# HamidGadirov/OpticalFlowSciVis

Measured on AMD Instinct MI355X. Metric: volume-pairs/sec, Flow-3D unsupervised train step (fwd+loss+bwd+AdamW), higher is better.
Workload: dtype f32

## Files before the change

### opticalflowscivis_amd/csrc/convtr.hip

```cpp
#include <cstdint>
#include <cstdlib>

#include "common.hpp"

namespace {

typedef float f32x16 __attribute__((ext_vector_type(16)));

struct TP {
  int B, Cin, Cout;
  int CoutT;
  int Di, Hi, Wi;
  int Dout, Hout, Wout;
  int Dq, Hq, Wq;
  int tz, ty, tx;
  long long tiles;
  const float* slope;
  float* Z;
  int nslope;
  const float* addend;
  const float* Ybase;
  long long wslice;
#ifdef FS_ABLATION
  int ab = 0;
// ... 568 lines not shown
#pragma unroll
    for (int cls = 0; cls < 8; ++cls) {
      const int pz = cls >> 2, py = (cls >> 1) & 1, px = cls & 1;
#pragma unroll
      for (int tp = 0; tp < 8; ++tp) {
        const int a = tp >> 2, bb = (tp >> 1) & 1, c = tp & 1;
        const int kidx = (tap_k(pz, a) * 4 + tap_k(py, bb)) * 4 + tap_k(px, c);
        const int didx = ((tap_d(pz, a) + 1) * 3 + (tap_d(py, bb) + 1)) * 3 + (tap_d(px, c) + 1);
        const float av = aB[kidx * 16];
#pragma unroll
        for (int n = 0; n < 2; ++n)
          acc[n][cls] = __builtin_amdgcn_mfma_f32_16x16x4f32(av, xn[n][didx], acc[n][cls], 0, 0, 0);
      }
    }
    __builtin_amdgcn_s_barrier();
    buf ^= 1;
  }

#ifdef FS_ABLATION
  if (p.ab & 4) return;
#endif
  const int qz = qz0 + wz, qy = qy0 + wy;
  if (qz < p.Dq && qy < p.Hq) {
    const size_t yvol = (size_t)p.Dout * p.Hout * p.Wout;
#pragma unroll
    for (int n = 0; n < 2; ++n) {
      const int qx = qx0 + 16 * n + col;
#pragma unroll
      for (int r = 0; r < 4; ++r) {
        const int co = 4 * kq + r;
        const bool ok = co < p.Cout;
        const int cc = ok ? co : 0;
        const float bv = (bias && ok) ? bias[cc] : 0.f;
        float v[8];
#pragma unroll
        for (int c = 0; c < 8; ++c) v[c] = acc[n][c][r] + bv;
        store8_quad(Y + ((size_t)b * p.Cout + cc) * yvol, v, qz, qy, qx, ok, p,
                    p.Z ? p.Z + ((size_t)b * p.Cout + cc) * yvol : nullptr, p.Z ? p.slope[p.nslope == 1 ? 0 : cc] : 0.f);
      }
    }
  }
}

constexpr int p8_ws_ci(int rt) { return 128 * rt + 16; }
__host__ __device__ constexpr int p8_k(int par, int d) { return par == 0 ? (d == 0 ? 1 : 3) : (d == 0 ? 0 : 2); }

#ifdef FS_TR_STAMPS
__device__ unsigned long long fs_tr_dbg[4 * 8];
#define TSTAMP(i) do { const unsigned long long now_ = __builtin_amdgcn_s_memtime(); dt[i] += now_ - tprev; tprev = now_; } while (0)
#else
#define TSTAMP(i) do { } while (0)
#endif

template <int RT, int NT, int CINP>
__global__ __launch_bounds__(512, 2) void convtr_p8_kernel(const float* __restrict__ X, const float* __restrict__ Wt,
                                                        const float* __restrict__ bias, float* __restrict__ Y,
                                                        TP p, int per) {
  constexpr int CI = 4, XB = 16 * (NT - 1);
  constexpr int ZT = 3, YT = 3, XP = XB + 16;
  constexpr int PS = YT * XP;
  constexpr int CHS = ZT * PS + ((ZT * PS) % 32 == 16 ? 0 : 16);
  constexpr int NX = CI * CHS;
  constexpr int NXL = (NX + 255) / 256 * 256;
  constexpr int WSCI = p8_ws_ci(RT);
  constexpr int NW = CINP * WSCI;
  constexpr int NWL = (NW + 255) / 256 * 256;
  static_assert((NWL + 2 * NXL) * 4 <= 160 * 1024, "weights + two input buffers fit the CU's LDS");
  static_assert(NT % 2 == 1, "tiles are processed in pairs + one");
  __shared__ __attribute__((aligned(16))) float lds[NWL + 2 * NXL];

  const int t = threadIdx.x, lane = t & 63;
  const int wave = __builtin_amdgcn_readfirstlane(t >> 6);
  const int wv = wave & 3;
  const long long t0 = (long long)blockIdx.x * per, t1 = min(t0 + per, p.tiles);
  const size_t xvol = (size_t)p.Di * p.Hi * p.Wi;
  auto decode = [&](long long tile, int& b, int& qz0, int& qy0, int& q0) {
    const int txi = (int)(tile % p.tx); tile /= p.tx;
    const int tyi = (int)(tile % p.ty); tile /= p.ty;
    const int tzi = (int)(tile % p.tz);
    b = (int)(tile / p.tz);
    qz0 = tzi * 2; qy0 = tyi * 2; q0 = txi * XB;
  };

  if (wave >= 4) {
#if defined(__HIP_DEVICE_COMPILE__)
    __builtin_amdgcn_s_setprio(3);
    constexpr int NXW = (NXL / 256 + 3) / 4, NWW = (NWL / 256 + 3) / 4;
    {
      __amdgpu_buffer_rsrc_t rw = __builtin_amdgcn_make_buffer_rsrc((void*)Wt, (short)0, (p.Cin + 3) / 4 * 4 * WSCI * 4,
                                                                     0x00020000);
#pragma unroll
      for (int k = 0; k < NWW; ++k)
        if (256 * (wv + 4 * k) < NWL)
          __builtin_amdgcn_raw_ptr_buffer_load_lds(rw, (lds_ptr_t)(lds + 256 * (wv + 4 * k)), 16,
                                                   (unsigned)(256 * (wv + 4 * k) + 4 * lane) * 4u, 0, 0, 0);
    }
    unsigned xoff[NXW];
    int b = 0;
    auto offsets = [&](long long tile) {
      int qz0, qy0, q0;
      decode(tile, b, qz0, qy0, q0);
#pragma unroll
      for (int k = 0; k < NXW; ++k) {
        const int i = 256 * (wv + 4 * k) + 4 * lane;
        const int c = i / CHS, r1 = i - c * CHS;
        const int z = r1 / PS, r2 = r1 - z * PS;
        const int y = r2 / XP, x = r2 - y * XP;
        const int gz = qz0 - 1 + z, gy = qy0 - 1 + y, gx = q0 - 4 + x;
        const bool ok = i < NX && z < ZT && gz >= 0 && gz < p.Di && gy >= 0 && gy < p.Hi && gx >= 0 && gx < p.Wi;
        xoff[k] = ok ? ((unsigned)c * (unsigned)xvol + ((unsigned)gz * p.Hi + gy) * p.Wi + gx) * 4u : DMA_OOB;
// ... 47 lines not shown
  for (long long tile = t0; tile < t1; ++tile) {
    int b, qz0, qy0, q0;
    decode(tile, b, qz0, qy0, q0);
    const int qend = (q0 + XB >= p.Wi) ? p.Wi + 1 : q0 + XB;
    f32x4 acc[RT][NT];
#pragma unroll
    for (int rt = 0; rt < RT; ++rt)
#pragma unroll
      for (int n = 0; n < NT; ++n)
#pragma unroll
        for (int r = 0; r < 4; ++r) acc[rt][n][r] = 0.f;

    for (int c0 = 0; c0 < p.Cin; c0 += CI) {
      const float* aB = lds + (size_t)(c0 + kq) * WSCI + col;
      float av[8][RT];
#pragma unroll
      for (int d = 0; d < 8; ++d)
#pragma unroll
        for (int rt = 0; rt < RT; ++rt) av[d][rt] = aB[(d * RT + rt) * 16];
      const float* bB = lds + bBo + buf * NXL;
      float xa[2][8], xb[2][8];
      auto load_x = [&](int n, float (&xn)[8]) {
#pragma unroll
        for (int d = 0; d < 8; ++d) xn[d] = bB[16 * n - ((d >> 2) & 1) * PS - ((d >> 1) & 1) * XP - (d & 1)];
      };
      auto mma_pair = [&](int n, const float (&x0)[8], const float (&x1)[8], bool two) {
#pragma unroll
        for (int d = 0; d < 8; ++d)
#pragma unroll
          for (int rt = 0; rt < RT; ++rt) {
            acc[rt][n] = __builtin_amdgcn_mfma_f32_16x16x4f32(av[d][rt], x0[d], acc[rt][n], 0, 0, 0);
            if (two) acc[rt][n + 1] = __builtin_amdgcn_mfma_f32_16x16x4f32(av[d][rt], x1[d], acc[rt][n + 1], 0, 0, 0);
          }
      };
      load_x(0, xa[0]);
      if (NT > 1) load_x(1, xa[1]);
#pragma unroll
      for (int n = 0; n < NT; n += 4) {
        if (n + 2 < NT) { load_x(n + 2, xb[0]); if (n + 3 < NT) load_x(n + 3, xb[1]); }
        __builtin_amdgcn_sched_barrier(0);
        mma_pair(n, xa[0], xa[1], n + 1 < NT);
        if (n + 2 < NT) {
          if (n + 4 < NT) { load_x(n + 4, xa[0]); if (n + 5 < NT) load_x(n + 5, xa[1]); }
          __builtin_amdgcn_sched_barrier(0);
          mma_pair(n + 2, xb[0], xb[1], n + 3 < NT);
        }
      }
      TSTAMP(0);
      __builtin_amdgcn_s_barrier();
      TSTAMP(1);
      buf ^= 1;
    }

    const int qz = qz0 + wz, qy = qy0 + wy;
    if (qz <= p.Di && qy <= p.Hi) {
      const size_t yvol = (size_t)p.Dout * p.Hout * p.Wout;
      const bool evn = (col & 1) == 0;
      const int slot = 4 * (kq & 1) + (evn ? 0 : 1) + 2 * (lane >> 5);
#pragma unroll
      for (int rt = 0; rt < RT; ++rt) {
        const int item = 8 * rt + slot;
        const int pzy = item / p.Cout, co = item - pzy * p.Cout;
        const int zo = 2 * qz - (pzy >> 1), yo = 2 * qy - (pzy & 1);
        const bool iok = item < 4 * p.Cout && zo >= 0 && zo < p.Dout && yo >= 0 && yo < p.Hout;
        const float bv = (bias && iok) ? bias[co] : 0.f;
        float* __restrict__ row = Y + (((size_t)b * p.Cout + (iok ? co : 0)) * p.Dout + (iok ? zo : 0)) * ((size_t)p.Hout * p.Wout) +
                                  (size_t)(iok ? yo : 0) * p.Wout;
        const float* __restrict__ arow = p.addend ? p.addend + (row - Y) : nullptr;
        (void)yvol;
        float4 apre[NT];
        if (arow != nullptr) {
#pragma unroll
          for (int n = 0; n < NT; ++n) {
            const int qa = evn ? q0 + 16 * n + col : q0 + 16 * n + col - 1;
            const int x0 = 2 * qa - 1;
            const bool full = iok && qa >= 1 && qa + 1 < qend && x0 + 3 < p.Wout;
            apre[n] = full ? *reinterpret_cast<const float4*>(arow + x0) : make_float4(0.f, 0.f, 0.f, 0.f);
          }
        }
#pragma unroll
        for (int n = 0; n < NT; ++n) {
          const int q = q0 + 16 * n + col;
          const auto s0 = __builtin_amdgcn_permlane32_swap(__float_as_uint(acc[rt][n][0]), __float_as_uint(acc[rt][n][2]),
                                                           false, false);
          const auto s1 = __builtin_amdgcn_permlane32_swap(__float_as_uint(acc[rt][n][1]), __float_as_uint(acc[rt][n][3]),
                                                           false, false);
          const unsigned keep_e = evn ? s0[0] : s1[0], keep_o = evn ? s0[1] : s1[1];
          const unsigned send_e = evn ? s1[0] : s0[0], send_o = evn ? s1[1] : s0[1];
          const float re = __uint_as_float(__builtin_amdgcn_update_dpp(0u, send_e, 0xB1, 0xF, 0xF, false)) + bv;
          const float ro = __uint_as_float(__builtin_amdgcn_update_dpp(0u, send_o, 0xB1, 0xF, 0xF, false)) + bv;
          const float ke = __uint_as_float(keep_e) + bv, ko = __uint_as_float(keep_o) + bv;
          const int qa = evn ? q : q - 1;
          float4 v = evn ? make_float4(ko, ke, ro, re) : make_float4(ro, re, ko, ke);
          if (iok) {
            const int x0 = 2 * qa - 1;
            const bool full = qa >= 1 && qa + 1 < qend && x0 + 3 < p.Wout;
            if (full) {
              if (arow) { v.x += apre[n].x; v.y += apre[n].y; v.z += apre[n].z; v.w += apre[n].w; }
              *reinterpret_cast<float4*>(row + x0) = v;
            } else {
              const float vv[4] = {v.x, v.y, v.z, v.w};
#pragma unroll
              for (int e = 0; e < 4; ++e) {
                const int x = x0 + e, pos = qa + (e >> 1);
                if (pos >= 0 && pos < qend && x >= 0 && x < p.Wout) row[x] = vv[e] + (arow ? arow[x] : 0.f);
              }
            }
          }
        }
      }
    }
    TSTAMP(2);
  }
#ifdef FS_TR_STAMPS
  if (blockIdx.x == 3 && lane == 0) {
    for (int i = 0; i < 8; ++i) fs_tr_dbg[wv * 8 + i] = dt[i];
    fs_tr_dbg[wv * 8 + 7] = (unsigned long long)(t1 - t0);
  }
#endif
}

static int tr_ncu() {
  static int ncu_of[64] = {};
  int dev = 0;
  if (hipGetDevice(&dev) != hipSuccess || dev < 0 || dev >= 64) dev = 0;
  int ncu = ncu_of[dev];
  if (ncu == 0) {
    int n = 0;
    if (hipDeviceGetAttribute(&n, hipDeviceAttributeMultiprocessorCount, dev) != hipSuccess || n < 1) n = 256;
    ncu_of[dev] = ncu = n;
  }
  return ncu;
}

template <int RT, int NT, int CINP = 32>
void launch_p8(const float* x, const float* ws, const float* bias, float* y, const TP& p, hipStream_t st) {
  const int ncu = tr_ncu();
  const long long nwg = p.tiles < ncu ? p.tiles : ncu;
  const int per = (int)((p.tiles + nwg - 1) / nwg);
  const unsigned grid = (unsigned)((p.tiles + per - 1) / per);
  hipLaunchKernelGGL((convtr_p8_kernel<RT, NT, CINP>), dim3(grid), dim3(512), 0, st, x, ws, bias, y, p, per);
}

template <int CO, int NP>
__global__ __launch_bounds__(256) void convtr_valu_kernel(const float* __restrict__ X, const float* __restrict__ W,
                                                          const float* __restrict__ bias, float* __restrict__ Y,
                                                          TP p) {
  const int Hq2 = (p.Hq + NP - 1) / NP;
  const long long nq = (long long)p.B * p.Dq * Hq2 * p.Wq;
  const long long e = (long long)blockIdx.x * 256 + threadIdx.x;
  if (e >= nq) return;
  const int qx = (int)(e % p.Wq);
  long long r = e / p.Wq;
  const int qy = (int)(r % Hq2) * NP; r /= Hq2;
  const int qz = (int)(r % p.Dq);
  const int b = (int)(r / p.Dq);

  constexpr int NY = NP + 2;
  int off[3 * NY * 3];
#pragma unroll
  for (int dz = 0; dz < 3; ++dz)
#pragma unroll
    for (int dy = 0; dy < NY; ++dy)
#pragma unroll
      for (int dx = 0; dx < 3; ++dx) {
        const int z = qz + dz - 1, y = qy + dy - 1, x = qx + dx - 1;
        const bool ok = z >= 0 && z < p.Di && y >= 0 && y < p.Hi && x >= 0 && x < p.Wi;
        off[(dz * NY + dy) * 3 + dx] = ok ? (z * p.Hi + y) * p.Wi + x : -1;
      }

  float acc[NP][CO][8];
#pragma unroll
// ... 13 lines not shown
    const float* wc = W + (size_t)ci * p.Cout * 64;
#pragma unroll
    for (int co = 0; co < CO; ++co) {
      if (co < p.Cout) {
#pragma unroll
        for (int cls = 0; cls < 8; ++cls) {
          const int pz = cls >> 2, py = (cls >> 1) & 1, px = cls & 1;
#pragma unroll
          for (int tp = 0; tp < 8; ++tp) {
            const int a = tp >> 2, bb = (tp >> 1) & 1, c = tp & 1;
            const int kidx = (tap_k(pz, a) * 4 + tap_k(py, bb)) * 4 + tap_k(px, c);
            const float wv = wc[co * 64 + kidx];
#pragma unroll
            for (int q = 0; q < NP; ++q) {
              const int didx = ((tap_d(pz, a) + 1) * NY + (tap_d(py, bb) + 1 + q)) * 3 + (tap_d(px, c) + 1);
              acc[q][co][cls] = fmaf(xn[didx], wv, acc[q][co][cls]);
            }
          }
        }
      }
    }
  }
  const size_t yvol = (size_t)p.Dout * p.Hout * p.Wout;
#pragma unroll
  for (int q = 0; q < NP; ++q)
#pragma unroll
    for (int co = 0; co < CO; ++co)
      if (co < p.Cout && qy + q < p.Hq)
        store8(Y + ((size_t)b * p.Cout + co) * yvol, acc[q][co], qz, qy + q, qx, p,
               p.Z ? p.Z + ((size_t)b * p.Cout + co) * yvol : nullptr, p.Z ? p.slope[p.nslope == 1 ? 0 : co] : 0.f);
}

template <int CO>
void launch_valu(const float* x, const float* w, const float* bias, float* y, const TP& p, hipStream_t st) {
  constexpr int NP = 2;
  const long long nq = (long long)p.B * p.Dq * ((p.Hq + NP - 1) / NP) * p.Wq;
  hipLaunchKernelGGL((convtr_valu_kernel<CO, NP>), dim3((unsigned)((nq + 255) / 256)), dim3(256), 0, st, x, w, bias,
                     y, p);
}

}

#ifdef FS_TR_STAMPS
extern "C" int fs_debug_tr_stamps(unsigned long long* out) {
  return hipMemcpyFromSymbol(out, HIP_SYMBOL(fs_tr_dbg), sizeof(unsigned long long) * 32) == hipSuccess ? 0 : 1;
}
#endif

extern "C" long long fs_conv3d_tr_ws_floats(int Cin, int Cout) {
  if (Cin < 1 || Cout < 1 || (Cout > 32 && (Cout % 32 != 0 || Cout > 128))) return -1;
  const int slices = Cout > 32 ? Cout / 32 : 1;
  if (Cout > 32) Cout = 32;
  const long long cinp = (Cin + 3) / 4 * 4;
  const long long p8 = Cout <= 12 ? cinp * p8_ws_ci(Cout <= 2 ? 1 : (Cout <= 6 ? 3 : 6)) : 0;
  long long cls = Cout <= 6 ? 0 : cinp * 64 * (Cout <= 16 ? 16 : 32);
  if (Cout > 16 && t3_slab_words(Cin) > cls) cls = t3_slab_words(Cin);
  if (Cout <= 16 && t3_slab_words16(Cin) > cls) cls = t3_slab_words16(Cin);
  return (p8 > cls ? p8 : cls) * slices;
}

static int conv3d_tr_slice(const float* x, const float* w, const float* bias, const float* slope, int nslope,
                          const float* addend, float* y, float* z, float* ws, int B, int Cin, int Cout, int Di,
                          int Hi, int Wi, int Dout, int Hout, int Wout, fs_stream_t stream, int CoutT = 0, int slices = 1,
                          WprepPlan* plan = nullptr) {
  FS_REQUIRE_PTR(x);
  if (plan == nullptr) FS_REQUIRE_PTR(y);
  if (z != nullptr && (slope == nullptr || (nslope != 1 && nslope != Cout))) return FS_ERR_ARG;
  if (B < 1 || Cin < 1 || Cout < 1 || Di < 1 || Hi < 1 || Wi < 1) return FS_ERR_SHAPE;
  if (Cout > 32) return FS_ERR_ARG;
  if (CoutT == 0) CoutT = Cout;
  if ((Dout != 2 * Di && Dout != 2 * Di + 1) || (Hout != 2 * Hi && Hout != 2 * Hi + 1) ||
      (Wout != 2 * Wi && Wout != 2 * Wi + 1))
    return FS_ERR_SHAPE;
  if ((long long)Di * Hi * Wi >= (1ll << 31) || (long long)Dout * Hout * Wout >= (1ll << 31))
    return FS_ERR_SHAPE;
  if ((long long)4 * Di * Hi * Wi * 4 >= (1ll << 32)) return FS_ERR_SHAPE;
  TP p;
  p.B = B; p.Cin = Cin; p.Cout = Cout; p.CoutT = CoutT; p.Di = Di; p.Hi = Hi; p.Wi = Wi;
  p.Dout = Dout; p.Hout = Hout; p.Wout = Wout;
  p.Dq = (Dout + 1) / 2; p.Hq = (Hout + 1) / 2; p.Wq = (Wout + 1) / 2;
  p.slope = slope; p.Z = z; p.nslope = nslope;
  p.addend = addend; p.Ybase = y;
  p.wslice = 0;
  hipStream_t st = (hipStream_t)stream;
  if ((long long)B * p.Dq * p.Hq * p.Wq >= (1ll << 31) * 256) return FS_ERR_SHAPE;
  static const bool reg_only = FS_AB_ENV("FLOWSCI_TR_REG");
  static const bool p8_all = FS_AB_ENV("FLOWSCI_TR_P8_ALL");
  static const bool s3_small = FS_AB_ENV("FLOWSCI_TR_S3_SMALL");
  if (!s3_small && Cout <= (p8_all ? 12 : 6) && !reg_only && z == nullptr && ws != nullptr && Cin <= (Cout <= 6 ? 64 : 32) && Dout == 2 * Di && Hout == 2 * Hi &&
      Wout == 2 * Wi && Wi % 4 == 0 && (((uintptr_t)x | (uintptr_t)ws) & 15) == 0 &&
      (long long)4 * Di * Hi * Wi * 4 < (1ll << 31)) {
    const int rt = Cout <= 2 ? 1 : (Cout <= 6 ? 3 : 6);
    const bool wide = Wi > 64 && rt < 6;
    p.tz = fs::cdiv(Di + 1, 2); p.ty = fs::cdiv(Hi + 1, 2); p.tx = fs::cdiv(Wi, wide ? 128 : 64);
    p.tiles = (long long)B * p.tz * p.ty * p.tx;
    if (p.tiles >= 16 && p.tiles < (1ll << 31)) {
      const int cinp = (Cin + 3) / 4 * 4;
      wprep_do(wprep_job(FS_WPREP_P8, w, ws, (long long)cinp * p8_ws_ci(rt), Cin, Cout, cinp, rt), plan, st);
      if (plan != nullptr) return FS_OK;
      if (Cin > 32) {
        if (rt == 1) { if (wide) launch_p8<1, 9, 64>(x, ws, bias, y, p, st); else launch_p8<1, 5, 64>(x, ws, bias, y, p, st); }
        else { if (wide) launch_p8<3, 9, 64>(x, ws, bias, y, p, st); else launch_p8<3, 5, 64>(x, ws, bias, y, p, st); }
      } else if (rt == 1) { if (wide) launch_p8<1, 9>(x, ws, bias, y, p, st); else launch_p8<1, 5>(x, ws, bias, y, p, st); }
      else if (rt == 3) { if (wide) launch_p8<3, 9>(x, ws, bias, y, p, st); else launch_p8<3, 5>(x, ws, bias, y, p, st); }
      else launch_p8<6, 5>(x, ws, bias, y, p, st);
      FS_LAUNCH_CHECK();
      return FS_OK;
    }
  }
  if (Cout <= 6 && !s3_small) {
    if (plan != nullptr) return FS_OK;
    if (w == nullptr) return FS_ERR_NULLPTR;
    if (Cout == 1) launch_valu<1>(x, w, bias, y, p, st);
    else if (Cout <= 2) launch_valu<2>(x, w, bias, y, p, st);
    else if (Cout <= 4) launch_valu<4>(x, w, bias, y, p, st);
    else launch_valu<6>(x, w, bias, y, p, st);
    FS_LAUNCH_CHECK();
    return FS_OK;
  }
  FS_REQUIRE_PTR(ws);
  const int cinp = (Cin + 3) / 4 * 4;
  p.tz = fs::cdiv(p.Dq, 2); p.ty = fs::cdiv(p.Hq, 2); p.tx = fs::cdiv(p.Wq, 32);
  p.tiles = (long long)B * p.tz * p.ty * p.tx;
  if (p.tiles >= (1ll << 31)) return FS_ERR_SHAPE;
#ifdef FS_ABLATION
  static const int tr_ab = (int)FS_AB_ENV_LL("FLOWSCI_TR_AB", 0);
  p.ab = tr_ab;
#endif
  const bool ws_ok = !reg_only && Wi % 4 == 0 && (((uintptr_t)x | (uintptr_t)ws) & 15) == 0 && p.tiles * slices >= 128 &&
                     (long long)4 * Di * Hi * Wi * 4 < (1ll << 31);
  static const bool no_s3 = FS_AB_ENV("FLOWSCI_TR_NO_S3");
  const long long t3 = (long long)B * fs::cdiv(Di, T3_TZ) * fs::cdiv(Hi, T3_TY) * fs::cdiv(Wi, T3_TW);
  const bool t3_ok = !no_s3 && !reg_only && Dout == 2 * Di && Hout == 2 * Hi && Wout == 2 * Wi && Wi % 4 == 0 &&
                     (((uintptr_t)x | (uintptr_t)ws) & 15) == 0 && (long long)Di * Hi * Wi * 4 < (1ll << 31) &&
                     t3 * slices >= 256 && t3 < (1ll << 31) && (long long)32 * Dout * Hout * Wout * 4 < (1ll << 32);
  if (Cout <= 16) {
    if (t3_ok && slices == 1) {
      wprep_do(wprep_job(FS_WPREP_TRS3_16, w, ws, t3_slab_words16(Cin), Cin, Cout, (Cin + 3) / 4, p.CoutT), plan, st);
      if (plan != nullptr) return FS_OK;
      p.tz = fs::cdiv(Di, T3_TZ); p.ty = fs::cdiv(Hi, T3_TY); p.tx = fs::cdiv(Wi, T3_TW);
      p.tiles = t3;
      const int ncu = tr_ncu();
      const long long gx = ncu < p.tiles ? ncu : p.tiles;
      hipLaunchKernelGGL(convtr_s3_kernel<true>, dim3((unsigned)gx, 1), dim3(64 * (T3_NMW + T3_NLW)), 0, st, x,
                         reinterpret_cast<const unsigned*>(ws), bias, y, p);
      FS_LAUNCH_CHECK();
      return FS_OK;
    }
    wprep_do(wprep_job(FS_WPREP_TR16, w, ws, (long long)cinp * 64 * 16, Cin, Cout, cinp), plan, st);
    if (plan != nullptr) return FS_OK;
    if (ws_ok)
// ... 85 lines not shown
```

### opticalflowscivis_amd/csrc/wprep.hpp

```cpp
#pragma once

enum { FS_WPREP_FWD = 0, FS_WPREP_TR32 = 1, FS_WPREP_TR16 = 2, FS_WPREP_P8 = 3, FS_WPREP_WINO = 4, FS_WPREP_WINO4 = 5,
       FS_WPREP_WINO2D = 6, FS_WPREP_S3K4 = 7, FS_WPREP_TRS3 = 8, FS_WPREP_TRS3_16 = 9 };

__device__ __forceinline__ unsigned s3_pack(float a, float b) {
  typedef __bf16 bf16x2_t __attribute__((ext_vector_type(2)));
  const bf16x2_t h = {(__bf16)a, (__bf16)b};
  return __builtin_bit_cast(unsigned, h);
}

__device__ __forceinline__ unsigned wprep_s3_word(const FsWprepJob& j, int e) {
  const int Cout = j.p[0], Cin = j.p[1], CinP2 = j.p[2], CP = j.p[3];
  const float* __restrict__ w = j.w;
  const int kx = e & 3;
  int r = e >> 2;
  const int col = r % CP; r /= CP;
  const int kh = r & 1, kyp = (r >> 1) & 1; r >>= 2;
  const int piece = r % 3; r /= 3;
  const int kz = r & 3; r >>= 2;
  const int cp = r % CinP2, mg = r / CinP2;
  const int co = mg * CP + col, tap = (kz * 4 + 2 * kyp + kh) * 4 + kx;
  float v[2];
#pragma unroll
  for (int i = 0; i < 2; ++i) {
    const int ci = 2 * cp + i;
    float a = (co < Cout && ci < Cin) ? w[((size_t)co * Cin + ci) * 64 + tap] : 0.f;
    for (int q = 0; q < piece; ++q) a = a - (float)(__bf16)a;
    v[i] = a;
  }
  return s3_pack(v[0], v[1]);
}
__host__ __device__ constexpr int wprep_p8_k(int par, int d) { return par == 0 ? (d == 0 ? 1 : 3) : (d == 0 ? 0 : 2); }

__device__ __forceinline__ unsigned wprep_t3_word(const FsWprepJob& j, int e) {
  const int Cin = j.p[0], Cout = j.p[1], CoutT = j.p[3];
  const float* __restrict__ w = j.w;
  const int c2 = e & 1, dxa = (e >> 1) & 1, co = (e >> 2) & 31, kh = (e >> 7) & 1;
  int r = e >> 8;
  const int piece = r % 3; r /= 3;
  const int az = r & 1, cls = (r >> 1) & 7, st = r >> 4;
  const int pz = cls >> 2, py = (cls >> 1) & 1, px = cls & 1;
  const int tap = (wprep_p8_k(pz, az) * 4 + wprep_p8_k(py, kh)) * 4 + wprep_p8_k(px, 1 - dxa);
  float v[2];
#pragma unroll
  for (int i = 0; i < 2; ++i) {
    const int ci = 4 * st + 2 * c2 + i;
    float a = (co < Cout && ci < Cin) ? w[((size_t)ci * CoutT + co) * 64 + tap] : 0.f;
    for (int q = 0; q < piece; ++q) a = a - (float)(__bf16)a;
    v[i] = a;
  }
  return s3_pack(v[0], v[1]);
}
__device__ __forceinline__ unsigned wprep_t3_word16(const FsWprepJob& j, int e) {
  const int Cin = j.p[0], Cout = j.p[1], CoutT = j.p[3];
  const float* __restrict__ w = j.w;
  const int c2 = e & 1, az = (e >> 1) & 1, co = (e >> 2) & 15, kq = (e >> 6) & 3;
  int r = e >> 8;
  const int piece = r % 3; r /= 3;
  const int cls = r & 7, st = r >> 3;
  const int pz = cls >> 2, py = (cls >> 1) & 1, px = cls & 1;
  const int tap = (wprep_p8_k(pz, az) * 4 + wprep_p8_k(py, kq >> 1)) * 4 + wprep_p8_k(px, kq & 1);
  float v[2];
#pragma unroll
  for (int i = 0; i < 2; ++i) {
    const int ci = 4 * st + 2 * c2 + i;
    float a = (co < Cout && ci < Cin) ? w[((size_t)ci * CoutT + co) * 64 + tap] : 0.f;
    for (int q = 0; q < piece; ++q) a = a - (float)(__bf16)a;
    v[i] = a;
  }
  return s3_pack(v[0], v[1]);
}
constexpr int FS_WINO_UCH = 9 * 4 * 64 + 16;
constexpr int FS_WINO4_UCH = 9 * 6 * 64;
constexpr int FS_WINO2D_UCH = 3 * 24 * 64;

__device__ __forceinline__ float wprep_g43(const float (&g)[3], int tt) {
  switch (tt) {
    case 0: return 0.25f * g[0];
    case 1: return (-1.f / 6.f) * ((g[0] + g[2]) + g[1]);
    case 2: return (-1.f / 6.f) * ((g[0] + g[2]) - g[1]);
    case 3: return (1.f / 24.f) * g[0] + ((1.f / 12.f) * g[1] + (1.f / 6.f) * g[2]);
    case 4: return (1.f / 24.f) * g[0] + ((-1.f / 12.f) * g[1] + (1.f / 6.f) * g[2]);
    default: return g[2];
  }
}
// ... 16 lines not shown
    }
    case FS_WPREP_TR16: {
      const int Cin = j.p[0], Cout = j.p[1];
      const int co = e & 15, tap = (e >> 4) & 63, ci = e >> 10;
      return (co < Cout && ci < Cin) ? w[((size_t)ci * Cout + co) * 64 + tap] : 0.f;
    }
    case FS_WPREP_WINO: {
      const int Cout = j.p[0], Cin = j.p[1], mode = j.p[3];
      const int ci = e / FS_WINO_UCH, i = e - ci * FS_WINO_UCH;
      if (i >= 9 * 4 * 64 || ci >= Cin) return 0.f;
      const int kk = i >> 8, tt = (i >> 6) & 3, co = i & 63;
      if (co >= Cout) return 0.f;
      float g[3];
#pragma unroll
      for (int kx = 0; kx < 3; ++kx)
        g[kx] = mode ? w[((size_t)ci * Cout + co) * 27 + (26 - (kk * 3 + kx))] : w[((size_t)co * Cin + ci) * 27 + kk * 3 + kx];
      return tt == 0 ? g[0] : tt == 1 ? 0.5f * ((g[0] + g[1]) + g[2]) : tt == 2 ? 0.5f * ((g[0] - g[1]) + g[2]) : g[2];
    }
    case FS_WPREP_WINO4: {
      const int Cout = j.p[0], Cin = j.p[1], mode = j.p[3];
      const int ci = e / FS_WINO4_UCH, i = e - ci * FS_WINO4_UCH;
      if (ci >= Cin) return 0.f;
      const int kk = i / 384, r = i - kk * 384;
      const int tt = r >> 6, co = r & 63;
      if (co >= Cout) return 0.f;
      float g[3];
#pragma unroll
      for (int kx = 0; kx < 3; ++kx)
        g[kx] = mode ? w[((size_t)ci * Cout + co) * 27 + (26 - (kk * 3 + kx))] : w[((size_t)co * Cin + ci) * 27 + kk * 3 + kx];
      return wprep_g43(g, tt);
    }
    case FS_WPREP_WINO2D: {
      const int Cout = j.p[0], Cin = j.p[1], mode = j.p[3];
      const int ci = e / FS_WINO2D_UCH, i = e - ci * FS_WINO2D_UCH;
      if (ci >= Cin) return 0.f;
      const int kz = i / 1536, r = i - kz * 1536;
      const int ty = r / 384, r2 = r - ty * 384;
      const int tx = r2 >> 6, co = r2 & 63;
      if (co >= Cout) return 0.f;
      float u[3];
#pragma unroll
      for (int ky = 0; ky < 3; ++ky) {
        float g[3];
#pragma unroll
        for (int kx = 0; kx < 3; ++kx) {
          const int tap = (kz * 3 + ky) * 3 + kx;
          g[kx] = mode ? w[((size_t)ci * Cout + co) * 27 + (26 - tap)] : w[((size_t)co * Cin + ci) * 27 + tap];
        }
        u[ky] = wprep_g43(g, tx);
      }
      return ty == 0 ? u[0] : ty == 1 ? 0.5f * ((u[0] + u[1]) + u[2]) : ty == 2 ? 0.5f * ((u[0] - u[1]) + u[2]) : u[2];
    }
    default: {
      const int Cin = j.p[0], Cout = j.p[1], RT = j.p[3];
      const int wsci = 128 * RT + 16;
      const int ci = e / wsci, i = e - ci * wsci;
      if (i >= 128 * RT || ci >= Cin) return 0.f;
      const int d = i / (16 * RT), r2 = i - d * 16 * RT;
      const int rt = r2 >> 4, row = r2 & 15;
      const int px = row >> 3, item = 8 * rt + (row & 7);
      if (item >= 4 * Cout) return 0.f;
      const int pzy = item / Cout, co = item - pzy * Cout;
      const int kz = wprep_p8_k(pzy >> 1, (d >> 2) & 1), ky = wprep_p8_k(pzy & 1, (d >> 1) & 1), kx = wprep_p8_k(px, d & 1);
      return w[((size_t)ci * Cout + co) * 64 + (kz * 4 + ky) * 4 + kx];
    }
  }
}

__device__ __forceinline__ void wprep_wino2d_blocks(const FsWprepJob& j, int first, int stride) {
  __shared__ float g9[64 * 9 + 64];
  const int Cout = j.p[0], Cin = j.p[1], CinP = j.p[2], mode = j.p[3];
  const float* __restrict__ w = j.w;
  const int t = threadIdx.x;
  for (int blk = first; blk < CinP * 3; blk += stride) {
    const int ci = blk / 3, kz = blk - ci * 3;
    __syncthreads();
    for (int i = t; i < 64 * 9; i += 256) {
      const int co = i / 9, k9 = i - co * 9;
      const int tap = kz * 9 + k9;
      float v = 0.f;
      if (co < Cout && ci < Cin) v = mode ? w[((size_t)ci * Cout + co) * 27 + (26 - tap)] : w[((size_t)co * Cin + ci) * 27 + tap];
      g9[co * 10 + k9] = v;
    }
    __syncthreads();
    const int co = t & 63, q = t >> 6;
    float* __restrict__ dst = j.ws + (size_t)ci * FS_WINO2D_UCH + kz * 1536 + co;
#pragma unroll
    for (int k = 0; k < 6; ++k) {
      const int e = 6 * q + k, ty = e / 6, tx = e - ty * 6;
      float u[3];
#pragma unroll
      for (int ky = 0; ky < 3; ++ky) {
        const float g[3] = {g9[co * 10 + ky * 3], g9[co * 10 + ky * 3 + 1], g9[co * 10 + ky * 3 + 2]};
        u[ky] = wprep_g43(g, tx);
      }
      const float v = ty == 0 ? u[0] : ty == 1 ? 0.5f * ((u[0] + u[1]) + u[2]) : ty == 2 ? 0.5f * ((u[0] - u[1]) + u[2]) : u[2];
      dst[ty * 384 + tx * 64] = (co < Cout && ci < Cin) ? v : 0.f;
    }
  }
}

__global__ __launch_bounds__(256) void wprep_one_kernel(FsWprepJob j) {
  if (j.kind == FS_WPREP_WINO2D && j.total == j.p[2] * FS_WINO2D_UCH) {
    wprep_wino2d_blocks(j, blockIdx.x, gridDim.x);
    return;
  }
  if (j.kind == FS_WPREP_S3K4 || j.kind == FS_WPREP_TRS3 || j.kind == FS_WPREP_TRS3_16) {
    for (int e = blockIdx.x * 256 + threadIdx.x; e < j.total; e += gridDim.x * 256)
      reinterpret_cast<unsigned*>(j.ws)[e] = j.kind == FS_WPREP_S3K4 ? wprep_s3_word(j, e)
                                             : (j.kind == FS_WPREP_TRS3 ? wprep_t3_word(j, e) : wprep_t3_word16(j, e));
    return;
  }
  for (int e = blockIdx.x * 256 + threadIdx.x; e < j.total; e += gridDim.x * 256) j.ws[e] = wprep_elem(j, e);
}

__global__ __launch_bounds__(256) void wprep_batch_kernel(const FsWprepJob* __restrict__ jobs) {
  const FsWprepJob j = jobs[blockIdx.y];
  if (j.kind == FS_WPREP_WINO2D && j.total == j.p[2] * FS_WINO2D_UCH) {
    wprep_wino2d_blocks(j, blockIdx.x, gridDim.x);
    return;
  }
  if (j.kind == FS_WPREP_S3K4 || j.kind == FS_WPREP_TRS3 || j.kind == FS_WPREP_TRS3_16) {
    for (int e = blockIdx.x * 256 + threadIdx.x; e < j.total; e += gridDim.x * 256)
      reinterpret_cast<unsigned*>(j.ws)[e] = j.kind == FS_WPREP_S3K4 ? wprep_s3_word(j, e)
                                             : (j.kind == FS_WPREP_TRS3 ? wprep_t3_word(j, e) : wprep_t3_word16(j, e));
    return;
  }
  for (int e = blockIdx.x * 256 + threadIdx.x; e < j.total; e += gridDim.x * 256) j.ws[e] = wprep_elem(j, e);
}

inline FsWprepJob wprep_job(int kind, const float* w, float* ws, long long total, int p0, int p1, int p2 = 0, int p3 = 0,
                            int p4 = 0, int p5 = 0) {
  FsWprepJob j;
  j.w = w; j.ws = ws; j.kind = kind; j.total = (int)total;
  j.p[0] = p0; j.p[1] = p1; j.p[2] = p2; j.p[3] = p3; j.p[4] = p4; j.p[5] = p5;
  return j;
}

struct WprepPlan { FsWprepJob* jobs; int cap; int n; };
inline void wprep_do(const FsWprepJob& j, WprepPlan* plan, hipStream_t st) {
  if (plan != nullptr) {
    if (plan->n < plan->cap) plan->jobs[plan->n] = j;
    plan->n++;
    return;
  }
  if (j.w == nullptr) return;
  hipLaunchKernelGGL(wprep_one_kernel, dim3((j.total + 255) / 256), dim3(256), 0, st, j);
}
```

Before: 29.72.

## Add bf16x3 split-precision MFMA path for p8 transposed conv with producer waves

For the p8 transposed-conv kernel with RT==3 and Cin<=32, adds a body that splits f32 inputs and weights into three bf16 pieces and runs bf16 MFMA over six piece products, keeping near-f32 accuracy. The kernel is specialised into four producer waves and four compute waves. Producer waves DMA input tiles into an LDS staging area, convert them to bf16 pieces and double-buffer them, while compute waves issue the MFMAs. Weight prep gains a matching bf16-piece layout, and the store epilogue is factored into a shared helper. The bf16 MFMA rate is meant to replace the slower f32 MFMA path, at the cost of more MFMA issues, more LDS, conversion work and a small precision difference.

```diff
diff --git a/opticalflowscivis_amd/csrc/convtr.hip b/opticalflowscivis_amd/csrc/convtr.hip
--- a/opticalflowscivis_amd/csrc/convtr.hip
+++ b/opticalflowscivis_amd/csrc/convtr.hip
@@ -644,10 +644,72 @@
 #define TSTAMP(i) do { } while (0)
 #endif
 
+template <int RT, int NT>
+__device__ __forceinline__ void p8_store(const f32x4 (&acc)[RT][NT], const float* __restrict__ bias, float* __restrict__ Y,
+                                         const TP& p, int b, int qz, int qy, int q0, int qend, int lane) {
+  const int col = lane & 15, kq = lane >> 4;
+  if (qz <= p.Di && qy <= p.Hi) {
+    const size_t yvol = (size_t)p.Dout * p.Hout * p.Wout;
+    const bool evn = (col & 1) == 0;
+    const int slot = 4 * (kq & 1) + (evn ? 0 : 1) + 2 * (lane >> 5);
+#pragma unroll
+    for (int rt = 0; rt < RT; ++rt) {
+      const int item = 8 * rt + slot;
+      const int pzy = item / p.Cout, co = item - pzy * p.Cout;
+      const int zo = 2 * qz - (pzy >> 1), yo = 2 * qy - (pzy & 1);
+      const bool iok = item < 4 * p.Cout && zo >= 0 && zo < p.Dout && yo >= 0 && yo < p.Hout;
+      const float bv = (bias && iok) ? bias[co] : 0.f;
+      float* __restrict__ row = Y + (((size_t)b * p.Cout + (iok ? co : 0)) * p.Dout + (iok ? zo : 0)) * ((size_t)p.Hout * p.Wout) +
+                                (size_t)(iok ? yo : 0) * p.Wout;
+      const float* __restrict__ arow = p.addend ? p.addend + (row - Y) : nullptr;
+      (void)yvol;
+      float4 apre[NT];
+      if (arow != nullptr) {
+#pragma unroll
+        for (int n = 0; n < NT; ++n) {
+          const int qa = evn ? q0 + 16 * n + col : q0 + 16 * n + col - 1;
+          const int x0 = 2 * qa - 1;
+          const bool full = iok && qa >= 1 && qa + 1 < qend && x0 + 3 < p.Wout;
+          apre[n] = full ? *reinterpret_cast<const float4*>(arow + x0) : make_float4(0.f, 0.f, 0.f, 0.f);
+        }
+      }
+#pragma unroll
+      for (int n = 0; n < NT; ++n) {
+        const int q = q0 + 16 * n + col;
+        const auto s0 = __builtin_amdgcn_permlane32_swap(__float_as_uint(acc[rt][n][0]), __float_as_uint(acc[rt][n][2]),
+                                                         false, false);
+        const auto s1 = __builtin_amdgcn_permlane32_swap(__float_as_uint(acc[rt][n][1]), __float_as_uint(acc[rt][n][3]),
+                                                         false, false);
+        const unsigned keep_e = evn ? s0[0] : s1[0], keep_o = evn ? s0[1] : s1[1];
+        const unsigned send_e = evn ? s1[0] : s0[0], send_o = evn ? s1[1] : s0[1];
+        const float re = __uint_as_float(__builtin_amdgcn_update_dpp(0u, send_e, 0xB1, 0xF, 0xF, false)) + bv;
+        const float ro = __uint_as_float(__builtin_amdgcn_update_dpp(0u, send_o, 0xB1, 0xF, 0xF, false)) + bv;
+        const float ke = __uint_as_float(keep_e) + bv, ko = __uint_as_float(keep_o) + bv;
+        const int qa = evn ? q : q - 1;
+        float4 v = evn ? make_float4(ko, ke, ro, re) : make_float4(ro, re, ko, ke);
+        if (iok) {
+          const int x0 = 2 * qa - 1;
+          const bool full = qa >= 1 && qa + 1 < qend && x0 + 3 < p.Wout;
+          if (full) {
+            if (arow) { v.x += apre[n].x; v.y += apre[n].y; v.z += apre[n].z; v.w += apre[n].w; }
+            *reinterpret_cast<float4*>(row + x0) = v;
+          } else {
+            const float vv[4] = {v.x, v.y, v.z, v.w};
+#pragma unroll
+            for (int e = 0; e < 4; ++e) {
+              const int x = x0 + e, pos = qa + (e >> 1);
+              if (pos >= 0 && pos < qend && x >= 0 && x < p.Wout) row[x] = vv[e] + (arow ? arow[x] : 0.f);
+            }
+          }
+        }
+      }
+    }
+  }
+}
+
 template <int RT, int NT, int CINP>
-__global__ __launch_bounds__(512, 2) void convtr_p8_kernel(const float* __restrict__ X, const float* __restrict__ Wt,
-                                                        const float* __restrict__ bias, float* __restrict__ Y,
-                                                        TP p, int per) {
+__device__ __forceinline__ void p8_f32_body(const float* __restrict__ X, const float* __restrict__ Wt,
+                                            const float* __restrict__ bias, float* __restrict__ Y, const TP& p, int per) {
   constexpr int CI = 4, XB = 16 * (NT - 1);
   constexpr int ZT = 3, YT = 3, XP = XB + 16;
   constexpr int PS = YT * XP;
@@ -801,64 +863,7 @@
       buf ^= 1;
     }
 
-    const int qz = qz0 + wz, qy = qy0 + wy;
-    if (qz <= p.Di && qy <= p.Hi) {
-      const size_t yvol = (size_t)p.Dout * p.Hout * p.Wout;
-      const bool evn = (col & 1) == 0;
-      const int slot = 4 * (kq & 1) + (evn ? 0 : 1) + 2 * (lane >> 5);
-#pragma unroll
-      for (int rt = 0; rt < RT; ++rt) {
-        const int item = 8 * rt + slot;
-        const int pzy = item / p.Cout, co = item - pzy * p.Cout;
-        const int zo = 2 * qz - (pzy >> 1), yo = 2 * qy - (pzy & 1);
-        const bool iok = item < 4 * p.Cout && zo >= 0 && zo < p.Dout && yo >= 0 && yo < p.Hout;
-        const float bv = (bias && iok) ? bias[co] : 0.f;
-        float* __restrict__ row = Y + (((size_t)b * p.Cout + (iok ? co : 0)) * p.Dout + (iok ? zo : 0)) * ((size_t)p.Hout * p.Wout) +
-                                  (size_t)(iok ? yo : 0) * p.Wout;
-        const float* __restrict__ arow = p.addend ? p.addend + (row - Y) : nullptr;
-        (void)yvol;
-        float4 apre[NT];
-        if (arow != nullptr) {
-#pragma unroll
-          for (int n = 0; n < NT; ++n) {
-            const int qa = evn ? q0 + 16 * n + col : q0 + 16 * n + col - 1;
-            const int x0 = 2 * qa - 1;
-            const bool full = iok && qa >= 1 && qa + 1 < qend && x0 + 3 < p.Wout;
-            apre[n] = full ? *reinterpret_cast<const float4*>(arow + x0) : make_float4(0.f, 0.f, 0.f, 0.f);
-          }
-        }
-#pragma unroll
-        for (int n = 0; n < NT; ++n) {
-          const int q = q0 + 16 * n + col;
-          const auto s0 = __builtin_amdgcn_permlane32_swap(__float_as_uint(acc[rt][n][0]), __float_as_uint(acc[rt][n][2]),
-                                                           false, false);
-          const auto s1 = __builtin_amdgcn_permlane32_swap(__float_as_uint(acc[rt][n][1]), __float_as_uint(acc[rt][n][3]),
-                                                           false, false);
-          const unsigned keep_e = evn ? s0[0] : s1[0], keep_o = evn ? s0[1] : s1[1];
-          const unsigned send_e = evn ? s1[0] : s0[0], send_o = evn ? s1[1] : s0[1];
-          const float re = __uint_as_float(__builtin_amdgcn_update_dpp(0u, send_e, 0xB1, 0xF, 0xF, false)) + bv;
-          const float ro = __uint_as_float(__builtin_amdgcn_update_dpp(0u, send_o, 0xB1, 0xF, 0xF, false)) + bv;
-          const float ke = __uint_as_float(keep_e) + bv, ko = __uint_as_float(keep_o) + bv;
-          const int qa = evn ? q : q - 1;
-          float4 v = evn ? make_float4(ko, ke, ro, re) : make_float4(ro, re, ko, ke);
-          if (iok) {
-            const int x0 = 2 * qa - 1;
-            const bool full = qa >= 1 && qa + 1 < qend && x0 + 3 < p.Wout;
-            if (full) {
-              if (arow) { v.x += apre[n].x; v.y += apre[n].y; v.z += apre[n].z; v.w += apre[n].w; }
-              *reinterpret_cast<float4*>(row + x0) = v;
-            } else {
-              const float vv[4] = {v.x, v.y, v.z, v.w};
-#pragma unroll
-              for (int e = 0; e < 4; ++e) {
-                const int x = x0 + e, pos = qa + (e >> 1);
-                if (pos >= 0 && pos < qend && x >= 0 && x < p.Wout) row[x] = vv[e] + (arow ? arow[x] : 0.f);
-              }
-            }
-          }
-        }
-      }
-    }
+    p8_store<RT, NT>(acc, bias, Y, p, b, qz0 + wz, qy0 + wy, q0, qend, lane);
     TSTAMP(2);
   }
 #ifdef FS_TR_STAMPS
@@ -867,6 +872,16 @@
     fs_tr_dbg[wv * 8 + 7] = (unsigned long long)(t1 - t0);
   }
 #endif
+}
+
+#include "convtr_p8s.hpp"
+
+template <int RT, int NT, int CINP>
+__global__ __launch_bounds__(512, 2) void convtr_p8_kernel(const float* __restrict__ X, const float* __restrict__ Wt,
+                                                        const float* __restrict__ bias, float* __restrict__ Y,
+                                                        TP p, int per) {
+  if constexpr (p8_split(RT, CINP)) p8_split_body<RT, NT>(X, Wt, bias, Y, p, per);
+  else p8_f32_body<RT, NT, CINP>(X, Wt, bias, Y, p, per);
 }
 
 static int tr_ncu() {
@@ -986,7 +1001,7 @@
   const int slices = Cout > 32 ? Cout / 32 : 1;
   if (Cout > 32) Cout = 32;
   const long long cinp = (Cin + 3) / 4 * 4;
-  const long long p8 = Cout <= 12 ? cinp * p8_ws_ci(Cout <= 2 ? 1 : (Cout <= 6 ? 3 : 6)) : 0;
+  const long long p8 = Cout <= 12 ? p8_ws_words((int)cinp, Cout <= 2 ? 1 : (Cout <= 6 ? 3 : 6)) : 0;
   long long cls = Cout <= 6 ? 0 : cinp * 64 * (Cout <= 16 ? 16 : 32);
   if (Cout > 16 && t3_slab_words(Cin) > cls) cls = t3_slab_words(Cin);
   if (Cout <= 16 && t3_slab_words16(Cin) > cls) cls = t3_slab_words16(Cin);
@@ -1030,7 +1045,7 @@
     p.tiles = (long long)B * p.tz * p.ty * p.tx;
     if (p.tiles >= 16 && p.tiles < (1ll << 31)) {
       const int cinp = (Cin + 3) / 4 * 4;
-      wprep_do(wprep_job(FS_WPREP_P8, w, ws, (long long)cinp * p8_ws_ci(rt), Cin, Cout, cinp, rt), plan, st);
+      wprep_do(wprep_job(FS_WPREP_P8, w, ws, p8_ws_words(cinp, rt), Cin, Cout, cinp, rt), plan, st);
       if (plan != nullptr) return FS_OK;
       if (Cin > 32) {
         if (rt == 1) { if (wide) launch_p8<1, 9, 64>(x, ws, bias, y, p, st); else launch_p8<1, 5, 64>(x, ws, bias, y, p, st); }
diff --git a/opticalflowscivis_amd/csrc/convtr_p8s.hpp b/opticalflowscivis_amd/csrc/convtr_p8s.hpp
--- /dev/null
+++ b/opticalflowscivis_amd/csrc/convtr_p8s.hpp
@@ -0,0 +1,234 @@
+#pragma once
+
+template <int RT, int NT>
+__device__ __forceinline__ void p8_split_body(const float* __restrict__ X, const float* __restrict__ Wt,
+                                              const float* __restrict__ bias, float* __restrict__ Y, const TP& p, int per) {
+  constexpr int CI = 4, XB = 16 * (NT - 1), XP = XB + 16;
+  constexpr int NQ = XP / 4;
+  constexpr int ROWB = XP * 8, PIECEB = 9 * ROWB, INB = 3 * PIECEB;
+  constexpr int WCH = 3 * RT * 1024;
+  constexpr int WB = 8 * WCH;
+  constexpr int NITEMS = 9 * NQ;
+  constexpr int NIW = (NITEMS + 63) / 64, NIT = (NIW + 3) / 4;
+  constexpr int STGC = NIW * 1024, STGB = 4 * STGC;
+  constexpr int NWW = (WB / 1024 + 3) / 4;
+  static_assert(WB + 2 * INB + STGB <= 160 * 1024, "weights + two input stages + the staging area fit the CU's LDS");
+  static_assert(NT % 2 == 1, "tiles are processed in pairs + one");
+  __shared__ __attribute__((aligned(16))) unsigned char lds[WB + 2 * INB + STGB];
+
+  const int t = threadIdx.x, lane = t & 63;
+  const int wave = __builtin_amdgcn_readfirstlane(t >> 6);
+  const int wv = wave & 3;
+  const long long t0 = (long long)blockIdx.x * per, t1 = min(t0 + per, p.tiles);
+  const int NS = (p.Cin + 3) / 4;
+  const size_t xvol = (size_t)p.Di * p.Hi * p.Wi;
+  auto decode = [&](long long tile, int& b, int& qz0, int& qy0, int& q0) {
+    const int txi = (int)(tile % p.tx); tile /= p.tx;
+    const int tyi = (int)(tile % p.ty); tile /= p.ty;
+    const int tzi = (int)(tile % p.tz);
+    b = (int)(tile / p.tz);
+    qz0 = tzi * 2; qy0 = tyi * 2; q0 = txi * XB;
+  };
+
+  if (wave >= 4) {
+#if defined(__HIP_DEVICE_COMPILE__)
+    __builtin_amdgcn_s_setprio(3);
+    {
+      __amdgpu_buffer_rsrc_t rw = __builtin_amdgcn_make_buffer_rsrc((void*)Wt, (short)0, NS * WCH, 0x00020000);
+#pragma unroll
+      for (int k = 0; k < NWW; ++k)
+        if (wv + 4 * k < WB / 1024)
+          __builtin_amdgcn_raw_ptr_buffer_load_lds(rw, (lds_ptr_t)(lds + 1024 * (wv + 4 * k)), 16,
+                                                   (unsigned)(1024 * (wv + 4 * k) + 16 * lane), 0, 0, 0);
+    }
+    unsigned char* const stg = lds + WB + 2 * INB;
+    unsigned xoff[NIT];
+    int l_b = 0;
+    auto offsets = [&](long long tile) {
+      int qz0, qy0, q0;
+      decode(tile, l_b, qz0, qy0, q0);
+#pragma unroll
+      for (int k = 0; k < NIT; ++k) {
+        const int item = 64 * (wv + 4 * k) + lane;
+        const int row = item / NQ, jq = item - row * NQ;
+        const int z = row / 3, y = row - z * 3;
+        const int gz = qz0 - 1 + z, gy = qy0 - 1 + y, gx = q0 - 4 + 4 * jq;
+        const bool ok = item < NITEMS && gz >= 0 && gz < p.Di && gy >= 0 && gy < p.Hi && gx >= 0 && gx + 3 < p.Wi;
+        xoff[k] = ok ? (((unsigned)gz * (unsigned)p.Hi + (unsigned)gy) * (unsigned)p.Wi + (unsigned)gx) * 4u : DMA_OOB;
+      }
+    };
+    auto request = [&](int c0) {
+#pragma unroll
+      for (int c = 0; c < CI; ++c) {
+        const int ch = c0 + c;
+        __amdgpu_buffer_rsrc_t rx = __builtin_amdgcn_make_buffer_rsrc(
+            (void*)(X + ((size_t)l_b * p.Cin + (ch < p.Cin ? ch : 0)) * xvol), (short)0,
+            ch < p.Cin ? (int)((unsigned)xvol * 4u) : 0, 0x00020000);
+#pragma unroll
+        for (int k = 0; k < NIT; ++k)
+          if (wv + 4 * k < NIW)
+            __builtin_amdgcn_raw_ptr_buffer_load_lds(rx, (lds_ptr_t)(stg + c * STGC + 1024 * (wv + 4 * k)), 16, xoff[k], 0, 0, 0);
+      }
+    };
+    auto fetch = [&](t3_u32x4 (&ld)[NIT][4]) {
+#pragma unroll
+      for (int k = 0; k < NIT; ++k)
+        if (wv + 4 * k < NIW) {
+#pragma unroll
+          for (int c = 0; c < CI; ++c)
+            ld[k][c] = *reinterpret_cast<const t3_u32x4*>(stg + c * STGC + 1024 * (wv + 4 * k) + 16 * lane);
+        }
+    };
+    auto convert = [&](int buf, const t3_u32x4 (&ld)[NIT][4]) {
+#pragma unroll
+      for (int k = 0; k < NIT; ++k) {
+        const int item = 64 * (wv + 4 * k) + lane;
+        if (wv + 4 * k < NIW && item < NITEMS) {
+          const int row = item / NQ, jq = item - row * NQ;
+          unsigned char* dst = lds + WB + buf * INB + row * ROWB + jq * 32;
+          const unsigned u[4][4] = {{ld[k][0].x, ld[k][0].y, ld[k][0].z, ld[k][0].w}, {ld[k][1].x, ld[k][1].y, ld[k][1].z, ld[k][1].w},
+                                    {ld[k][2].x, ld[k][2].y, ld[k][2].z, ld[k][2].w}, {ld[k][3].x, ld[k][3].y, ld[k][3].z, ld[k][3].w}};
+          unsigned h[3][4][2];
+#pragma unroll
+          for (int i = 0; i < 4; ++i)
+#pragma unroll
+            for (int cp = 0; cp < 2; ++cp) {
+              float ra = __uint_as_float(u[2 * cp][i]), rc = __uint_as_float(u[2 * cp + 1][i]);
+              h[0][i][cp] = s3_pack(ra, rc);
+              ra -= __uint_as_float(h[0][i][cp] << 16); rc -= __uint_as_float(h[0][i][cp] & 0xffff0000u);
+              asm volatile("" : "+v"(ra), "+v"(rc));
+              h[1][i][cp] = s3_pack(ra, rc);
+              ra -= __uint_as_float(h[1][i][cp] << 16); rc -= __uint_as_float(h[1][i][cp] & 0xffff0000u);
+              asm volatile("" : "+v"(ra), "+v"(rc));
+              h[2][i][cp] = s3_pack(ra, rc);
+            }
+#pragma unroll
+          for (int pc = 0; pc < 3; ++pc) {
+            const t3_u32x4 v0 = {h[pc][0][0], h[pc][0][1], h[pc][1][0], h[pc][1][1]};
+            const t3_u32x4 v1 = {h[pc][2][0], h[pc][2][1], h[pc][3][0], h[pc][3][1]};
+            *reinterpret_cast<t3_u32x4*>(dst + pc * PIECEB) = v0;
+            *reinterpret_cast<t3_u32x4*>(dst + pc * PIECEB + 16) = v1;
+          }
+        }
+      }
+    };
+    const long long total = (t1 - t0) * NS;
+    long long l_tile = t0;
+    int l_s = 0;
+    auto advance = [&]() {
+      if (++l_s == NS) { l_s = 0; ++l_tile; offsets(l_tile); }
+    };
+    t3_u32x4 ld[NIT][4];
+    if (total > 0) {
+      offsets(t0);
+      request(0);
+    }
+    asm volatile("s_waitcnt vmcnt(0)" ::: "memory");
+    if (total > 0) {
+      fetch(ld);
+      asm volatile("s_waitcnt lgkmcnt(0)" ::: "memory");
+      __builtin_amdgcn_sched_barrier(0);
+      if (total > 1) { advance(); request(CI * l_s); }
+      __builtin_amdgcn_sched_barrier(0);
+      convert(0, ld);
+    }
+    asm volatile("s_waitcnt lgkmcnt(0)" ::: "memory");
+    __builtin_amdgcn_s_barrier();
+    for (long long g = 0; g < total; ++g) {
+      if (g + 1 < total) {
+        asm volatile("s_waitcnt vmcnt(0)" ::: "memory");
+        fetch(ld);
+        asm volatile("s_waitcnt lgkmcnt(0)" ::: "memory");
+        __builtin_amdgcn_sched_barrier(0);
+        if (g + 2 < total) { advance(); request(CI * l_s); }
+        __builtin_amdgcn_sched_barrier(0);
+        convert((int)((g + 1) & 1), ld);
+        asm volatile("s_waitcnt lgkmcnt(0)" ::: "memory");
+      }
+      __builtin_amdgcn_s_barrier();
+    }
+#else
+    (void)xvol; (void)NS; (void)NWW; (void)NIT; (void)STGB; (void)CI;
+#endif
+    return;
+  }
+
+  const int col = lane & 15, kq = lane >> 4;
+  const int wz = wv >> 1, wy = wv & 1;
+  const unsigned bO = (unsigned)(WB + ((wz + 1) * 3 + (wy + 1 - (kq >> 1))) * ROWB + (col + 4 - (kq & 1)) * 8);
+  __builtin_amdgcn_s_barrier();
+  int buf = 0;
+#ifdef FS_TR_STAMPS
+  unsigned long long dt[8] = {0, 0, 0, 0, 0, 0, 0, 0};
+  unsigned long long tprev = __builtin_amdgcn_s_memtime();
+#endif
+  for (long long tile = t0; tile < t1; ++tile) {
+    int b, qz0, qy0, q0;
+    decode(tile, b, qz0, qy0, q0);
+    const int qend = (q0 + XB >= p.Wi) ? p.Wi + 1 : q0 + XB;
+    f32x4 acc[RT][NT];
+#pragma unroll
+    for (int rt = 0; rt < RT; ++rt)
+#pragma unroll
+      for (int n = 0; n < NT; ++n)
+#pragma unroll
+        for (int r = 0; r < 4; ++r) acc[rt][n][r] = 0.f;
+
+    for (int s = 0; s < NS; ++s) {
+      const unsigned char* sw = lds + s * WCH + lane * 16;
+      t3_bf16x8 a[3][RT];
+#pragma unroll
+      for (int pc = 0; pc < 3; ++pc)
+#pragma unroll
+        for (int rt = 0; rt < RT; ++rt)
+          a[pc][rt] = __builtin_bit_cast(t3_bf16x8, *reinterpret_cast<const t3_u32x4*>(sw + (pc * RT + rt) * 1024));
+      const unsigned char* sb = lds + bO + buf * INB;
+      auto read_b = [&](int n, t3_bf16x8 (&bq)[3]) {
+#pragma unroll
+        for (int pc = 0; pc < 3; ++pc) {
+          const unsigned char* q = sb + pc * PIECEB + n * 128;
+          const t3_u32x2 lo = *(t3_lds_v64)(lds_ptr_t)(q), hi = *(t3_lds_v64)(lds_ptr_t)(q - 3 * ROWB);
+          const t3_u32x4 v = {lo.x, lo.y, hi.x, hi.y};
+          bq[pc] = __builtin_bit_cast(t3_bf16x8, v);
+        }
+      };
+      constexpr int PA[6] = {2, 0, 1, 1, 0, 0}, PB[6] = {0, 2, 1, 0, 1, 0};
+      auto mma_pair = [&](int n, const t3_bf16x8 (&x0)[3], const t3_bf16x8 (&x1)[3], bool two) {
+#pragma unroll
+        for (int q6 = 0; q6 < 6; ++q6)
+#pragma unroll
+          for (int rt = 0; rt < RT; ++rt) {
+            acc[rt][n] = __builtin_amdgcn_mfma_f32_16x16x32_bf16(a[PA[q6]][rt], x0[PB[q6]], acc[rt][n], 0, 0, 0);
+            if (two) acc[rt][n + 1] = __builtin_amdgcn_mfma_f32_16x16x32_bf16(a[PA[q6]][rt], x1[PB[q6]], acc[rt][n + 1], 0, 0, 0);
+          }
+      };
+      t3_bf16x8 xa[2][3], xb[2][3];
+      read_b(0, xa[0]);
+      if (NT > 1) read_b(1, xa[1]);
+#pragma unroll
+      for (int n = 0; n < NT; n += 4) {
+        if (n + 2 < NT) { read_b(n + 2, xb[0]); if (n + 3 < NT) read_b(n + 3, xb[1]); }
+        __builtin_amdgcn_sched_barrier(0);
+        mma_pair(n, xa[0], xa[1], n + 1 < NT);
+        if (n + 2 < NT) {
+          if (n + 4 < NT) { read_b(n + 4, xa[0]); if (n + 5 < NT) read_b(n + 5, xa[1]); }
+          __builtin_amdgcn_sched_barrier(0);
+          mma_pair(n + 2, xb[0], xb[1], n + 3 < NT);
+        }
+      }
+      TSTAMP(0);
+      __builtin_amdgcn_s_barrier();
+      TSTAMP(1);
+      buf ^= 1;
+    }
+
+    p8_store<RT, NT>(acc, bias, Y, p, b, qz0 + wz, qy0 + wy, q0, qend, lane);
+    TSTAMP(2);
+  }
+#ifdef FS_TR_STAMPS
+  if (blockIdx.x == 3 && lane == 0) {
+    for (int i = 0; i < 8; ++i) fs_tr_dbg[wv * 8 + i] = dt[i];
+    fs_tr_dbg[wv * 8 + 7] = (unsigned long long)(t1 - t0);
+  }
+#endif
+}
diff --git a/opticalflowscivis_amd/csrc/wprep.hpp b/opticalflowscivis_amd/csrc/wprep.hpp
--- a/opticalflowscivis_amd/csrc/wprep.hpp
+++ b/opticalflowscivis_amd/csrc/wprep.hpp
@@ -31,6 +31,34 @@
   return s3_pack(v[0], v[1]);
 }
 __host__ __device__ constexpr int wprep_p8_k(int par, int d) { return par == 0 ? (d == 0 ? 1 : 3) : (d == 0 ? 0 : 2); }
+
+__host__ __device__ constexpr bool p8_split(int rt, int cinp) { return cinp <= 32 && rt == 3; }
+__host__ __device__ constexpr long long p8_ws_words(int cinp, int rt) {
+  return p8_split(rt, cinp) ? (long long)cinp * 192 * rt : (long long)cinp * (128 * rt + 16);
+}
+__device__ __forceinline__ float wprep_p8_value(const FsWprepJob& j, int ci, int d, int rt, int row) {
+  const int Cin = j.p[0], Cout = j.p[1];
+  const int px = row >> 3, item = 8 * rt + (row & 7);
+  if (ci >= Cin || item >= 4 * Cout) return 0.f;
+  const int pzy = item / Cout, co = item - pzy * Cout;
+  const int kz = wprep_p8_k(pzy >> 1, (d >> 2) & 1), ky = wprep_p8_k(pzy & 1, (d >> 1) & 1), kx = wprep_p8_k(px, d & 1);
+  return j.w[((size_t)ci * Cout + co) * 64 + (kz * 4 + ky) * 4 + kx];
+}
+__device__ __forceinline__ unsigned wprep_p8s_word(const FsWprepJob& j, int e) {
+  const int RT = j.p[3];
+  const int c2 = e & 1, dz = (e >> 1) & 1, row = (e >> 2) & 15, kq = (e >> 6) & 3;
+  int r = e >> 8;
+  const int rt = r % RT; r /= RT;
+  const int piece = r % 3, chunk = r / 3;
+  float v[2];
+#pragma unroll
+  for (int i = 0; i < 2; ++i) {
+    float a = wprep_p8_value(j, 4 * chunk + 2 * c2 + i, 4 * dz + kq, rt, row);
+    for (int q = 0; q < piece; ++q) a = a - (float)(__bf16)a;
+    v[i] = a;
+  }
+  return s3_pack(v[0], v[1]);
+}
 
 __device__ __forceinline__ unsigned wprep_t3_word(const FsWprepJob& j, int e) {
   const int Cin = j.p[0], Cout = j.p[1], CoutT = j.p[3];
@@ -153,19 +181,23 @@
       return ty == 0 ? u[0] : ty == 1 ? 0.5f * ((u[0] + u[1]) + u[2]) : ty == 2 ? 0.5f * ((u[0] - u[1]) + u[2]) : u[2];
     }
     default: {
-      const int Cin = j.p[0], Cout = j.p[1], RT = j.p[3];
+      const int RT = j.p[3];
       const int wsci = 128 * RT + 16;
       const int ci = e / wsci, i = e - ci * wsci;
-      if (i >= 128 * RT || ci >= Cin) return 0.f;
+      if (i >= 128 * RT) return 0.f;
       const int d = i / (16 * RT), r2 = i - d * 16 * RT;
-      const int rt = r2 >> 4, row = r2 & 15;
-      const int px = row >> 3, item = 8 * rt + (row & 7);
-      if (item >= 4 * Cout) return 0.f;
-      const int pzy = item / Cout, co = item - pzy * Cout;
-      const int kz = wprep_p8_k(pzy >> 1, (d >> 2) & 1), ky = wprep_p8_k(pzy & 1, (d >> 1) & 1), kx = wprep_p8_k(px, d & 1);
-      return w[((size_t)ci * Cout + co) * 64 + (kz * 4 + ky) * 4 + kx];
-    }
-  }
+      return wprep_p8_value(j, ci, d, r2 >> 4, r2 & 15);
+    }
+  }
+}
+
+__device__ __forceinline__ bool wprep_bf16_words(const FsWprepJob& j) {
+  return j.kind == FS_WPREP_S3K4 || j.kind == FS_WPREP_TRS3 || j.kind == FS_WPREP_TRS3_16 ||
+         (j.kind == FS_WPREP_P8 && p8_split(j.p[3], j.p[2]));
+}
+__device__ __forceinline__ unsigned wprep_word(const FsWprepJob& j, int e) {
+  return j.kind == FS_WPREP_S3K4 ? wprep_s3_word(j, e)
+         : (j.kind == FS_WPREP_TRS3 ? wprep_t3_word(j, e) : (j.kind == FS_WPREP_TRS3_16 ? wprep_t3_word16(j, e) : wprep_p8s_word(j, e)));
 }
 
 __device__ __forceinline__ void wprep_wino2d_blocks(const FsWprepJob& j, int first, int stride) {
@@ -206,10 +238,9 @@
     wprep_wino2d_blocks(j, blockIdx.x, gridDim.x);
     return;
   }
-  if (j.kind == FS_WPREP_S3K4 || j.kind == FS_WPREP_TRS3 || j.kind == FS_WPREP_TRS3_16) {
+  if (wprep_bf16_words(j)) {
     for (int e = blockIdx.x * 256 + threadIdx.x; e < j.total; e += gridDim.x * 256)
-      reinterpret_cast<unsigned*>(j.ws)[e] = j.kind == FS_WPREP_S3K4 ? wprep_s3_word(j, e)
-                                             : (j.kind == FS_WPREP_TRS3 ? wprep_t3_word(j, e) : wprep_t3_word16(j, e));
+      reinterpret_cast<unsigned*>(j.ws)[e] = wprep_word(j, e);
     return;
   }
   for (int e = blockIdx.x * 256 + threadIdx.x; e < j.total; e += gridDim.x * 256) j.ws[e] = wprep_elem(j, e);
@@ -221,10 +252,9 @@
     wprep_wino2d_blocks(j, blockIdx.x, gridDim.x);
     return;
   }
-  if (j.kind == FS_WPREP_S3K4 || j.kind == FS_WPREP_TRS3 || j.kind == FS_WPREP_TRS3_16) {
+  if (wprep_bf16_words(j)) {
     for (int e = blockIdx.x * 256 + threadIdx.x; e < j.total; e += gridDim.x * 256)
-      reinterpret_cast<unsigned*>(j.ws)[e] = j.kind == FS_WPREP_S3K4 ? wprep_s3_word(j, e)
-                                             : (j.kind == FS_WPREP_TRS3 ? wprep_t3_word(j, e) : wprep_t3_word16(j, e));
+      reinterpret_cast<unsigned*>(j.ws)[e] = wprep_word(j, e);
     return;
   }
   for (int e = blockIdx.x * 256 + threadIdx.x; e < j.total; e += gridDim.x * 256) j.ws[e] = wprep_elem(j, e);
```

Result: no change. 29.95, median of 4 (+0.8%).
